# RM-Zhang/SGCDet

Hardware: AMD Instinct MI355X
Metric: scenes/sec (40-view ScanNet volume) at 1/2/4/8 MI355X; mAP@0.25 parity (higher is better)
Workload: dtype f32 (neck/head conv: 3xbf16-split MFMA, fp32 accumulate, ~1e-5 of fp32; wide 3x3x3 stride-1 layers through a Winograd F(2,3) transform along z: <= 2e-5 of the tensor scale per layer against the direct fp32 convolution); 1 GPU; cfg2_scannet: 40 views x 256 ch, images 256x320, FPN maps 64x80/32x40/16x20, D=12, voxels 40x40x16, top-k [800, 6400], neck 3-scale -> ScanNetImVoxelHeadV2; occupancy=predicted, masked_tail=False, input_layout=nchw, scenes_in_flight_per_gpu=4, launch=one hipGraph replay per scene (device-side pair counts, no host read-back)

## Files before the change

sgcdet_amd/csrc/conv3d.hip:

```cpp
#include "conv_common.hpp"
#include "tuning.hpp"

namespace sgc {
int g_conv_products = 3;


__global__ __launch_bounds__(256) void zero_fill_kernel(float4 *__restrict__ p, int64_t n4) {
  for (int64_t i = (int64_t)blockIdx.x * blockDim.x + threadIdx.x; i < n4; i += (int64_t)gridDim.x * blockDim.x)
    p[i] = make_float4(0.f, 0.f, 0.f, 0.f);
}
static int zero_fill(float *y, int64_t n, hipStream_t st) {
  const int64_t n4 = n / 4;
  const int g = (int)((n4 + 255) / 256 < 2048 ? (n4 + 255) / 256 : 2048);
  hipLaunchKernelGGL(zero_fill_kernel, dim3(g > 0 ? g : 1), dim3(256), 0, st, reinterpret_cast<float4 *>(y), n4);
  return check_launch("zero_fill_kernel");
}

static int halo_brick_shape(int gx, int gy, int gz) {
  if (g_tune_halo_brick == 2) return 2;
  if (g_tune_halo_brick == 0 && gz >= 16 && gx % 8 == 0 && gy % 8 == 0 && gz % 4 == 0) return 2;
  if (gz >= 16 && (g_tune_halo_brick == 0 || g_tune_halo_brick == 3)) return 0;
  if (gz >= 8) return 1;
  return 2;
}
// ... 134 lines not shown

static int pick_split_steps(const ConvParams &p, int mb, int nb, int target_blocks, int *steps_per) {
  const int total = (p.transposed ? 1 : p.taps) * (p.Cin / BK);
  *steps_per = total;
  if (p.two_d) return 1;
  if (!p.transposed && p.taps == 1) return 1;
  if (!g_tune_split_free) {
    const int k = pick_splitk(p, mb, nb, target_blocks);
    *steps_per = total / k;
    return k;
  }
  const int64_t tiles = (int64_t)mb * nb * (p.transposed ? 8 : 1);
  int64_t want = target_blocks / (tiles > 0 ? tiles : 1);
  if (want > total / g_tune_split_min_steps) want = total / g_tune_split_min_steps;
  if (want > g_tune_split_max) want = g_tune_split_max;
  if (want <= 1) return 1;
  const int per = (total + (int)want - 1) / (int)want;
  *steps_per = per;
  return (total + per - 1) / per;
}

static int conv_finish(const ConvParams &p, int64_t OV, hipStream_t st) {
  if (p.splitk <= 1) return SGC_OK;
  if (p.Cout % 4) return set_error(SGC_EUNSUP, "conv3d: split-K path needs Cout %% 4 == 0");
  const int64_t total4 = OV * p.Cout / 4;
  const int g = (int)((total4 + 255) / 256 < 4096 ? (total4 + 255) / 256 : 4096);
  hipLaunchKernelGGL(conv_epilogue_kernel, dim3(g), dim3(256), 0, st, p.y, p.scale, p.shift, p.residual, total4,
                     p.Cout / 4, p.relu, (const float *)p.ws, p.splitk, p.act_scale, p.act_c0, p.act_c1);
  return check_launch("conv_epilogue_kernel");
}

static ConvPlan plan_conv(const ConvParams &p, int64_t OV, bool masked) {
  ConvPlan pl = {};
  pl.family = kConvTile; pl.splitk = 1;
  const bool halo = g_tune_conv_halo && !p.transposed && p.ksize == 3 && p.stride == 1 && p.Cout >= g_tune_halo_min_cout;
  const bool narrow_n = g_tune_halo_narrow && p.Cout <= 64;
  const bool narrow_32 = g_tune_halo_narrow >= 1 && g_tune_halo_narrow != 64 && p.Cout <= 32;
  const auto brick = [&pl](ConvFamily f, int bx, int by, int bz, int bn) { pl.family = f; pl.bx = bx; pl.by = by; pl.bz = bz; pl.bn = bn; };
  int small = 0;
  if (!p.transposed && p.ksize == 1 && p.stride == 1 && !p.two_d && rows_gemm_supported(p.Cin, p.Cout, 0, 0, OV, p.Cin)) {
    pl.family = kConvRowsGemm;
    return pl;
  } else if (halo && !p.two_d && p.M >= g_tune_halo_min_m) {
    const int shape = halo_brick_shape(p.gx, p.gy, p.gz), bn = narrow_32 ? 32 : narrow_n ? 64 : 128;
    if (shape == 0) brick(kConvHalo, 4, 4, 16, bn);
    else if (shape == 1) brick(kConvHalo, 4, 8, 8, bn);
    else brick(kConvHalo, 8, 8, 4, bn);
  } else if (halo && !p.two_d && !masked && (small = halo_small_grid(p.gx, p.gy, p.gz, p.Cout)) != 0) {
    if (small == 1) brick(kConvHaloGrid, 10, 10, 4, 64);
    else brick(kConvHaloGrid, 6, 12, 4, 64);
  } else if (halo && g_tune_halo_2d && p.two_d && p.wz_Z > 0 && p.gy >= 8 && p.gz >= 8) {
    const int J = p.wz_Z / 2;
    const bool stack = !narrow_n && p.w_group_images == J && p.gx == 4 * J && p.wz_Z % 4 == 0;
    const bool fit4 = stack && J % 4 == 0 && p.M >= g_tune_halo_min_m, fit2 = stack && (J == 2 || fit4);
    const auto rows = [&p](int bx, int by, int bz) { return (int64_t)ceil_div(p.gx, bx) * ceil_div(p.gy, by) * ceil_div(p.gz, bz) * 256; };
    const bool small = fit2 && (!fit4 || g_tune_wz_brick == 2 || (g_tune_wz_brick == 0 && rows(2, 10, 10) < rows(4, 8, 8)));
    if (small) brick(kConvHaloWZ, 2, 10, 10, 128);
    else if (fit4) brick(kConvHaloWZ, 4, 8, 8, 128);
    if (pl.family == kConvHaloWZ && J % pl.bx != 0) pl.unsupported = "conv: a brick of the virtual Winograd stack must hold images of one position";
    else if (pl.family != kConvHaloWZ) pl.unsupported = "conv: the virtual Winograd stack needs Z / 2 = 2 or a multiple of 4 (and then halo_min_m stack rows) and > 64 output channels";
  } else if (halo && g_tune_halo_2d && p.two_d && p.wz_Z == 0 && p.M >= g_tune_halo_min_m && p.gy >= 8 && p.gz >= 8) {
    if ((g_tune_halo_2d == 2 || p.w_group_images > 0) && !narrow_n && p.gx % 4 == 0 && (p.w_group_images == 0 || p.w_group_images % 4 == 0))
      brick(kConvHalo2D, 4, 8, 8, 128);
    else if (p.w_group_images > 0) pl.unsupported = "conv: grouped 2-D form needs groups of a multiple of 4 images and > 64 output channels";
    else brick(kConvHalo2D, 1, 16, 16, narrow_n ? 64 : 128);
  } else if (p.w_group_images > 0 || p.wz_Z > 0) {
    pl.unsupported = "conv: the grouped 2-D form runs on the halo kernel only (stack too small?)";
  }
  if (pl.unsupported) return pl;
  if (pl.family == kConvTile) {
    pl.bn = p.Cout <= 64 ? 64 : 128;
    pl.splitk = pick_split_steps(p, ceil_div(p.M, BM), ceil_div(p.Cout, pl.bn), g_tune_split_target, &pl.steps_per);
  } else {
    pl.splitk = halo_splitk(ceil_div(p.gx, pl.bx) * ceil_div(p.gy, pl.by) * ceil_div(p.gz, pl.bz), ceil_div(p.Cout, pl.bn), p.Cin / BK);
    if (pl.family == kConvHaloWZ && p.M >= g_tune_halo_min_m) pl.splitk = 1;
  }
  pl.ws_floats = pl.splitk > 1 ? (int64_t)pl.splitk * OV * p.Cout : 0;
  return pl;
}

static int conv_split_begin(ConvParams &p, int64_t OV, hipStream_t st) {
  if (p.splitk <= 1) return SGC_OK;
  if (p.Cout % 4) return set_error(SGC_EUNSUP, "conv3d: split-K path needs Cout %% 4 == 0");
  if (p.ws && p.ws_floats >= (int64_t)p.splitk * OV * p.Cout) {
    p.ws_stride = OV * p.Cout;
    return SGC_OK;
  }
  p.ws = nullptr;
  return zero_fill(p.y, OV * p.Cout, st);
}

// ... 226 lines not shown
```

sgcdet_amd/csrc/conv3d_halo.hpp:

```cpp
#pragma once
#include "conv_common.hpp"
#include "mma.hpp"
#include "diag.hpp"
#include "tuning.hpp"

namespace sgc {

__host__ __device__ constexpr int halo_pitch(int BZ) { return BZ == 8 ? 12 : BZ == 10 ? 13 : BZ + 2; }
__host__ __device__ constexpr size_t halo_tab_offset(int lrows, int mrows = 256, int bnv = 128) {
  const size_t planes = (size_t)(2 * lrows + 2 * 2 * bnv) * LDKH * sizeof(uint16_t);
  const size_t stage = (size_t)mrows * (bnv + 8) * sizeof(float);
  return planes > stage ? planes : stage;
}

template <int BX, int BY, int BZ, int BNV = 128, int NP = 3, bool TD = false, bool STG = true, bool WZ = false>
__global__ __launch_bounds__(512) void conv3d_halo_bf16x3_kernel(const ConvParamsB p) {
  static_assert(!WZ || TD, "the virtual Winograd stack is a 2-D form");
  constexpr int NTAP = TD ? 9 : 27, XO = TD ? 0 : 1;
  constexpr int WNV = BNV >= 64 ? 2 : 1, WMV = 8 / WNV;
  constexpr int NVOX = BX * BY * BZ, MROWS = (NVOX + 32 * WMV - 1) / (32 * WMV) * (32 * WMV);
  constexpr int RT = MROWS / (32 * WMV);
  constexpr unsigned short kPadRow = 0x8000;
  static_assert(MROWS <= 512, "one table entry per thread");
  constexpr int TN = BNV / (32 * WNV), WCOL = BNV / WNV;
  constexpr int HX = BX + 2 * XO, HY = BY + 2, HZ = BZ + 2, HROWS = HX * HY * HZ;
  constexpr int HZP = halo_pitch(BZ), LROWS = HX * HY * HZP;
  constexpr int NT = 512;
  constexpr int NA = (HROWS * 8 + NT - 1) / NT;
  constexpr int A_PLANE = LROWS * LDKH, B_PLANE = BNV * LDKH;
  extern __shared__ __attribute__((aligned(16))) unsigned char smem_h[];
  __bf16 *A_hi = reinterpret_cast<__bf16 *>(smem_h), *A_lo = A_hi + A_PLANE;
  __bf16 *Bbase = A_lo + A_PLANE;
  unsigned short *vox_tab = reinterpret_cast<unsigned short *>(smem_h + halo_tab_offset(LROWS, MROWS, MROWS > 256 ? BNV : 128));

  const int tid = threadIdx.x, lane = tid & 63, wid = tid >> 6;
  const int wm = wid / WNV, wn = wid % WNV;
  const int nby = (p.gy + BY - 1) / BY, nbz = (p.gz + BZ - 1) / BZ;
  int bid = blockIdx.x;
  const int bk = bid % nbz; bid /= nbz;
  const int bj = bid % nby; const int bi = bid / nby;
  const int X0 = bi * BX, Y0 = bj * BY, Z0 = bk * BZ;
  const int n0 = blockIdx.y * BNV;
  const int nchunks = p.Cin / BK;
  const int per = (nchunks + p.splitk - 1) / p.splitk;
  const int c_lo = blockIdx.z * per, c_hi = min(nchunks, c_lo + per);
  if (c_lo >= c_hi) return;

  for (int t = wid; t < MROWS / 32; t += NT / 64) {
    const int j = lane & 31;
    const int r = t * 32 + j, rv = r < NVOX ? r : 0;
    const int x = rv / (BY * BZ), y = (rv / BZ) % BY, z = rv % BZ;
    const int res = (((x + XO) * HY + (y + 1)) * HZP + (z + 1)) & 15;
    unsigned same = 0, mine = 0;
#pragma unroll
    for (int q = 0; q < 16; ++q) {
      const unsigned m = (unsigned)__ballot(res == q);
      if (res == q) same = m;
      if ((j & 15) == q) mine = m;
    }
    const unsigned below = (1u << j) - 1u;
    const int rank = __popc(same & below);
    const bool slot_empty = __popc(mine) < (j >> 4) + 1;
    const unsigned left = (unsigned)__ballot(rank >= 2), empty = (unsigned)__ballot(slot_empty);
    const unsigned short val = r < NVOX ? (unsigned short)r : kPadRow;
    unsigned short *tab = vox_tab + t * 32, *tmp = vox_tab + MROWS + (wid & 7) * 32;
    if (lane < 32) {
      if (rank < 2) tab[rank * 16 + res] = val;
      else tmp[__popc(left & below)] = val;
    }
    asm volatile("s_waitcnt lgkmcnt(0)" ::: "memory");
    if (lane < 32 && slot_empty) tab[j] = tmp[__popc(empty & below)];
  }
  __syncthreads();
  const int fr = lane & 31, fh = lane >> 5;
  int arow[RT];
#pragma unroll
  for (int i = 0; i < RT; ++i) {
    const int r = vox_tab[(wm * RT + i) * 32 + fr] & 0x7fff;
    const int x = r / (BY * BZ), y = (r / BZ) % BY, z = r % BZ;
    arow[i] = ((x + XO) * HY + (y + 1)) * HZP + (z + 1);
  }
  bool wave_live = true;
  if (p.out_mask) {
    bool mine = false;
#pragma unroll
    for (int i = 0; i < RT; ++i) {
      const int r = vox_tab[(wm * RT + i) * 32 + fr];
      const int x = X0 + r / (BY * BZ), y = Y0 + (r / BZ) % BY, z = Z0 + r % BZ;
      if (!(r & kPadRow) && x < p.gx && y < p.gy && z < p.gz) mine |= p.out_mask[((int64_t)x * p.gy + y) * p.gz + z] != 0;
    }
    wave_live = __ballot(mine) != 0ull;
    if (!__syncthreads_or(wave_live ? 1 : 0)) {
      if (p.splitk > 1 && !p.ws) return;
      for (int e = tid; e < NVOX * (BNV / 4); e += NT) {
        const int rl = e / (BNV / 4), c4 = e - rl * (BNV / 4);
        const int col = n0 + c4 * 4;
        if (col >= p.Cout) continue;
        const int x = X0 + rl / (BY * BZ), y = Y0 + (rl / BZ) % BY, z = Z0 + rl % BZ;
        if (x >= p.gx || y >= p.gy || z >= p.gz) continue;
        const int64_t orow = ((int64_t)x * p.gy + y) * p.gz + z;
        for (int q = 0; q < 4 && col + q < p.Cout; ++q) {
          float v = 0.f;
          if (p.splitk > 1) { p.ws[(int64_t)blockIdx.z * p.ws_stride + orow * p.Cout + col + q] = 0.f; continue; }
          v = v * (p.scale ? p.scale[col + q] : 1.f) + (p.shift ? p.shift[col + q] : 0.f);
          if (p.relu == 2) v = relu_nan(v);
          if (p.residual) v += p.residual[orow * p.Cout + col + q];
          if (p.relu == 1) v = relu_nan(v);
          if (p.act_scale) v = act_col(v, col + q, p.act_c0, p.act_c1, *p.act_scale);
          p.y[orow * p.Cout + col + q] = v;
        }
      }
      return;
    }
  }
  const int bc = tid & 3, rs16 = (tid >> 2) & 15;
  const int bn = 16 * wid + (rs16 >> 2) + 4 * (rs16 & 3);
  const bool bn_ok = tid < BNV * 4 && n0 + bn < p.Cout;

  f32x16 acc[RT][TN];
#pragma unroll
  for (int i = 0; i < RT; ++i)
#pragma unroll
    for (int j = 0; j < TN; ++j)
#pragma unroll
      for (int k = 0; k < 16; ++k) acc[i][j][k] = 0.f;
  SGC_HALO_STAMP(0);

  float4 ra[NA], rw[WZ ? NA : 1];
  uint4 rbh, rbl;
  constexpr unsigned OOB = 0xfffffff0u;
  const __amdgpu_buffer_rsrc_t xr = __builtin_amdgcn_make_buffer_rsrc(
      const_cast<float *>(p.x), 0, (int)(unsigned)((int64_t)(WZ ? p.wz_Z : p.ix) * p.iy * p.iz * p.Cin * 4), 0x00020000);
  const int w_bytes = (int)(unsigned)((int64_t)NTAP * p.Cout * p.Cin * 2);
  const int64_t w_set = (TD && p.w_group_images > 0) ? (int64_t)(X0 / p.w_group_images) * NTAP * p.Cout * p.Cin : 0;
  const __amdgpu_buffer_rsrc_t whr = __builtin_amdgcn_make_buffer_rsrc(const_cast<__bf16 *>(p.w_hi + w_set), 0, w_bytes, 0x00020000);
  const __amdgpu_buffer_rsrc_t wlr = __builtin_amdgcn_make_buffer_rsrc(const_cast<__bf16 *>(p.w_lo + w_set), 0, w_bytes, 0x00020000);
  unsigned aoff[NA], aoffb[WZ ? NA : 1];
#pragma unroll
  for (int i = 0; i < NA; ++i) {
    const int idx = i * NT + tid;
    const int row = idx >> 3, c4 = idx & 7;
    const int hz = row % HZ, hy = (row / HZ) % HY, hx = row / (HZ * HY);
    const int gx = X0 + hx - XO, gy = Y0 + hy - 1, gz = Z0 + hz - 1;
    const bool in = row < HROWS && gx >= 0 && gx < p.ix && gy >= 0 && gy < p.iy && gz >= 0 && gz < p.iz;
    if constexpr (WZ) {
      const int J = p.wz_Z >> 1, kpos = X0 / J, j = gx - kpos * J;
      const int za = kpos == 0 ? 2 * j - 1 : kpos == 2 ? 2 * j + 1 : 2 * j;
      const int zb = kpos <= 1 ? 2 * j + 1 : kpos == 2 ? 2 * j : 2 * j + 2;
      const unsigned col = (unsigned)((gy * p.iz + gz) * p.wz_Z);
      aoff[i] = in && za >= 0 ? ((col + (unsigned)za) * (unsigned)p.Cin + c4 * 4) * 4u : OOB;
      aoffb[i] = in && zb < p.wz_Z ? ((col + (unsigned)zb) * (unsigned)p.Cin + c4 * 4) * 4u : OOB;
    } else {
      aoff[i] = in ? ((unsigned)((gx * p.iy + gy) * p.iz + gz) * (unsigned)p.Cin + c4 * 4) * 4u : OOB;
    }
  }
  const float wz_sign = WZ && (X0 / max(p.wz_Z >> 1, 1)) == 1 ? 1.f : -1.f;
  const unsigned boff = bn_ok ? (unsigned)((n0 + bn) * p.Cin + bc * 8) * 2u : OOB;
  auto load_A = [&](int cc) {
// ... 54 lines not shown
    const int dx = TD ? XO : tap / 9, dy = (tap / 3) % 3, dz = tap % 3;
    return ((dx - XO) * HY + (dy - 1)) * HZP + (dz - 1);
  };
  struct Frag { bf16x8 ah[RT], al[RT], bh[TN], bl[TN]; };
  auto read_A = [&](Frag &f, int toff, int kk) {
#pragma unroll
    for (int i = 0; i < RT; ++i) {
      const int o = (arow[i] + toff) * LDKH + fh * 8 + kk * 16;
      f.ah[i] = *reinterpret_cast<const bf16x8 *>(A_hi + o);
      if constexpr (NP == 3) f.al[i] = *reinterpret_cast<const bf16x8 *>(A_lo + o);
    }
  };
  auto read_B = [&](Frag &f, int buf, int kk) {
    const __bf16 *b = Bbase + buf * 2 * B_PLANE + (wn * WCOL + fr) * LDKH + fh * 8 + kk * 16;
#pragma unroll
    for (int j = 0; j < TN; ++j) {
      f.bh[j] = *reinterpret_cast<const bf16x8 *>(b + j * 32 * LDKH);
      if constexpr (NP == 3) f.bl[j] = *reinterpret_cast<const bf16x8 *>(b + B_PLANE + j * 32 * LDKH);
    }
  };
  auto mfma_half = [&](const Frag &f) {
    if constexpr ((SGC_HALO_SKIP & 32) != 0) {
#pragma unroll
      for (int i = 0; i < RT; ++i) asm volatile("" ::"v"(f.ah[i]), "v"(f.al[i]));
#pragma unroll
      for (int j = 0; j < TN; ++j) asm volatile("" ::"v"(f.bh[j]), "v"(f.bl[j]));
      return;
    }
#pragma unroll
    for (int i = 0; i < RT; ++i)
#pragma unroll
      for (int j = 0; j < TN; ++j) acc[i][j] = mma_split<NP>(f.ah[i], f.al[i], f.bh[j], f.bl[j], acc[i][j]);
  };
  const int steps_total = (c_hi - c_lo) * NTAP;
  auto step_tap = [&](int st) { return st % NTAP; };
  auto step_cc = [&](int st) { return c_lo + st / NTAP; };

  if constexpr (STG) {
    load_A(c_lo);
    load_B(0, c_lo);
    split_A();
    store_A();
    store_B(0);
    if (steps_total > 1) load_B(step_tap(1), step_cc(1));
    __syncthreads();
    Frag P = {}, Q = {};
    constexpr int SKIP = SGC_HALO_SKIP;
    if (wave_live) { read_A(P, tap_off(0), 0); read_B(P, 0, 0); }
    int g = 0;
    for (int cc = c_lo; cc < c_hi; ++cc) {
#pragma unroll
      for (int tap = 0; tap < NTAP; ++tap, ++g) {
        const bool last_tap = tap == NTAP - 1;
        const bool more = g + 1 < steps_total;
        if (wave_live) {
          if (!(SKIP & 16) || g == 0) read_A(Q, tap_off(tap), 1);
          if (!(SKIP & 8) || g == 0) read_B(Q, g & 1, 1);
        }
        if (!(SKIP & 2) && more) store_B((g + 1) & 1);
        if (!(SKIP & 4) && g + 2 < steps_total) load_B(step_tap(g + 2), step_cc(g + 2));
        if (!(SKIP & 64) && tap == NTAP - 3 && cc + 1 < c_hi) load_A(cc + 1);
        if (wave_live) mfma_half(P);
        if (!(SKIP & 64) && last_tap && cc + 1 < c_hi) split_A();
        if (!(SKIP & 1)) __syncthreads();
        __builtin_amdgcn_sched_barrier(0);
        if (wave_live && !last_tap) {
          if (!(SKIP & 16)) read_A(P, tap_off(tap + 1), 0);
          if (!(SKIP & 8)) read_B(P, (g + 1) & 1, 0);
        }
        if (!(SKIP & 64) && last_tap && cc + 1 < c_hi) store_A();
        if (wave_live) mfma_half(Q);
// ... 14 lines not shown
    store_B(0);
    __syncthreads();
    Frag P = {}, Q = {};
    read_A(P, tap_off(0), 0);
    for (int cc = c_lo; cc < c_hi; ++cc) {
      for (int tap = 0; tap < NTAP; ++tap, ++g) {
        const bool last_tap = tap == NTAP - 1;
        if (!(SKIP & 4) && g + 1 < steps_total) load_B(step_tap(g + 1), step_cc(g + 1));
        if (tap == NTAP - 3 && cc + 1 < c_hi) load_A(cc + 1);
        const int toff = tap_off(tap);
        if (wave_live) {
          if (!(SKIP & 8) || g == 0) read_B(P, g & 1, 0);
          if (!(SKIP & 16) || g == 0) read_A(Q, toff, 1);
          if (!(SKIP & 8) || g == 0) read_B(Q, g & 1, 1);
          mfma_half(P);
          mfma_half(Q);
          if (!last_tap && (!(SKIP & 16) || g == 0)) read_A(P, tap_off(tap + 1), 0);
        }
        if (!(SKIP & 2) && g + 1 < steps_total) store_B((g + 1) & 1);
        if (last_tap && cc + 1 < c_hi) split_A();
        if (!(SKIP & 1)) __syncthreads();
      }
      if (cc + 1 < c_hi) {
        store_A();
        __syncthreads();
        if (wave_live && (!(SKIP & 16))) read_A(P, tap_off(0), 0);
      }
    }
  }
  SGC_HALO_STAMP(2);
  if constexpr ((SGC_HALO_SKIP & 128) != 0) { if (p.relu != 77) return; }

  if ((p.Cout & 3) == 0 && (p.splitk == 1 || p.ws)) {
    constexpr int LDC = BNV + 8;
    float *cs = reinterpret_cast<float *>(smem_h);
    if constexpr (STG) __syncthreads();
#pragma unroll
    for (int i = 0; i < RT; ++i)
#pragma unroll
      for (int j = 0; j < TN; ++j)
#pragma unroll
        for (int k = 0; k < 16; ++k)
          cs[(wm * (RT * 32) + i * 32 + (k & 3) + 8 * (k >> 2) + 4 * (lane >> 5)) * LDC + wn * WCOL + j * 32 + (lane & 31)] = acc[i][j][k];
    __syncthreads();
    constexpr int C4 = BNV / 4;
    for (int e = tid; e < MROWS * C4; e += NT) {
      const int rl = e / C4, c4 = e - rl * C4;
      const int col = n0 + c4 * 4;
      if (col >= p.Cout) continue;
      const int r = vox_tab[rl];
      if (r & kPadRow) continue;
      const int x = X0 + r / (BY * BZ), y = Y0 + (r / BZ) % BY, z = Z0 + r % BZ;
      if (x >= p.gx || y >= p.gy || z >= p.gz) continue;
      const int64_t orow = ((int64_t)x * p.gy + y) * p.gz + z;
      float4 v = *reinterpret_cast<const float4 *>(cs + rl * LDC + c4 * 4);
      if (p.splitk > 1) {
        *reinterpret_cast<float4 *>(p.ws + (int64_t)blockIdx.z * p.ws_stride + orow * p.Cout + col) = v;
        continue;
      }
      if (p.scale) {
        const float4 sc4 = *reinterpret_cast<const float4 *>(p.scale + col);
        v.x *= sc4.x; v.y *= sc4.y; v.z *= sc4.z; v.w *= sc4.w;
      }
      if (p.shift) {
        const float4 sh4 = *reinterpret_cast<const float4 *>(p.shift + col);
        v.x += sh4.x; v.y += sh4.y; v.z += sh4.z; v.w += sh4.w;
      }
      if (p.relu == 2) v = relu_nan(v);
      if (p.residual) {
        const float4 r4 = *reinterpret_cast<const float4 *>(p.residual + orow * p.Cout + col);
        v.x += r4.x; v.y += r4.y; v.z += r4.z; v.w += r4.w;
      }
      if (p.relu == 1) v = relu_nan(v);
      if (p.act_scale) v = act_col4(v, col, p.act_c0, p.act_c1, *p.act_scale);
      *reinterpret_cast<float4 *>(p.y + orow * p.Cout + col) = v;
    }
    return;
  }

#pragma unroll
  for (int i = 0; i < RT; ++i)
#pragma unroll
    for (int j = 0; j < TN; ++j) {
      const int col = n0 + wn * WCOL + j * 32 + (lane & 31);
      if (col >= p.Cout) continue;
      const float sc = p.scale ? p.scale[col] : 1.f, sh = p.shift ? p.shift[col] : 0.f;
#pragma unroll
      for (int k = 0; k < 16; ++k) {
        const int r = vox_tab[(wm * RT + i) * 32 + (k & 3) + 8 * (k >> 2) + 4 * (lane >> 5)];
        const int x = X0 + r / (BY * BZ), y = Y0 + (r / BZ) % BY, z = Z0 + r % BZ;
        if ((r & kPadRow) || x >= p.gx || y >= p.gy || z >= p.gz) continue;
        const int64_t orow = ((int64_t)x * p.gy + y) * p.gz + z;
        float *dst = p.y + orow * p.Cout + col;
        if (p.splitk > 1) {
          if (p.ws) p.ws[(int64_t)blockIdx.z * p.ws_stride + orow * p.Cout + col] = acc[i][j][k];
          else atomicAdd(dst, acc[i][j][k]);
        } else {
          float v = acc[i][j][k] * sc + sh;
          if (p.relu == 2) v = relu_nan(v);
          if (p.residual) v += p.residual[orow * p.Cout + col];
          if (p.relu == 1) v = relu_nan(v);
          if (p.act_scale) v = act_col(v, col, p.act_c0, p.act_c1, *p.act_scale);
          *dst = v;
        }
      }
    }
}


template <int BX, int BY, int BZ, int BNV, int NP, bool TD, bool STG, bool WZ = false>
static int launch_halo_k(ConvParamsB &p, hipStream_t st) {
#if defined(SGC_HALO_STAMPS)
  p.stamps = g_halo_stamp_buf;
#endif
  constexpr int LROWS = (TD ? BX : BX + 2) * (BY + 2) * halo_pitch(BZ);
  constexpr int RGRAN = BNV >= 64 ? 128 : 256;
  constexpr int MROWS = (BX * BY * BZ + RGRAN - 1) / RGRAN * RGRAN;
  const size_t smem = halo_tab_offset(LROWS, MROWS, MROWS > 256 ? BNV : 128) + (MROWS + 256) * sizeof(uint16_t);
  static_assert(halo_tab_offset(LROWS, MROWS, MROWS > 256 ? BNV : 128) + (MROWS + 256) * sizeof(uint16_t) <= 160 * 1024, "brick does not fit the LDS");
  static std::atomic<uint64_t> attr_done{0};
  ensure_dynamic_lds((const void *)conv3d_halo_bf16x3_kernel<BX, BY, BZ, BNV, NP, TD, STG, WZ>, (int)smem, attr_done);
  const int bricks = ceil_div(p.gx, BX) * ceil_div(p.gy, BY) * ceil_div(p.gz, BZ);
  const int nb = ceil_div(p.Cout, BNV);
  hipLaunchKernelGGL((conv3d_halo_bf16x3_kernel<BX, BY, BZ, BNV, NP, TD, STG, WZ>), dim3(bricks, nb, p.splitk), dim3(512), smem, st, p);
  return check_launch("conv3d_halo_bf16x3_kernel");
}

template <int BX, int BY, int BZ, int BNV = 128, bool TD = false, bool WZ = false>
static int launch_halo(ConvParamsB &p, hipStream_t st) {
  if constexpr (!WZ) {
    if (g_conv_products == 3) {
      if (!g_tune_halo_stagger || BX * BY * BZ > 256) return launch_halo_k<BX, BY, BZ, BNV, 3, TD, false>(p, st);
      return launch_halo_k<BX, BY, BZ, BNV, 3, TD, true>(p, st);
    }
  }
  return with_products(g_conv_products, [&](auto np) { return launch_halo_k<BX, BY, BZ, BNV, np(), TD, true, WZ>(p, st); });
}

int launch_halo_z4(ConvParamsB &p, const ConvPlan &pl, hipStream_t st);
int launch_halo_2d(ConvParamsB &p, const ConvPlan &pl, hipStream_t st);
}
```

sgcdet_amd/csrc/conv3d_halo_2d.hip:

```cpp
#include "conv3d_halo.hpp"

namespace sgc {
int launch_halo_2d(ConvParamsB &p, const ConvPlan &pl, hipStream_t st) {
  if (pl.family == kConvHaloWZ)
    return pl.bx == 2 ? launch_halo<2, 10, 10, 128, true, true>(p, st) : launch_halo<4, 8, 8, 128, true, true>(p, st);
  if (pl.bx == 4) return launch_halo<4, 8, 8, 128, true>(p, st);
  return pl.bn == 64 ? launch_halo<1, 16, 16, 64, true>(p, st) : launch_halo<1, 16, 16, 128, true>(p, st);
}
}
```

sgcdet_amd/csrc/conv_common.hpp:

```cpp
#pragma once
#include "common.hpp"

namespace sgc {
extern int g_conv_products;

bool rows_gemm_supported(int K, int N, int hm_cm, int hm_S, int64_t rows, int64_t ldx);
int device_cus();
int rows_gemm_launch(const float *x, int64_t ldx, const uint16_t *w_hi, const uint16_t *w_lo, const float *scale,
                     const float *shift, const float *residual, void *y, const int32_t *m_dev, int M, int K, int N, int relu,
                     int hm_S, int hm_cm, int hm_bf16, hipStream_t st, float *zero_row = nullptr);
bool rows_gemm_gather_supported(int K, int N, int64_t x_rows, int64_t rows);
int rows_gemm_gather_launch(const float *x, int64_t x_rows, const float *gw, const int32_t *go, const uint16_t *w_hi, const uint16_t *w_lo,
                            const float *shift, float *y, const int32_t *m_dev, int M, int K, int N, hipStream_t st);

struct ConvParams {
  const float *x;
  const float *w;
  const float *scale;
  const float *shift;
  const float *residual;
  float *y;
  int Cin, Cout;
  int ix, iy, iz;
  int gx, gy, gz;
// ... 12 lines not shown
  int two_d;
  unsigned long long *stamps;
  int xcd_deal;
  int wz_Z;
  int w_group_images;
  float *zero_row;
  const float *act_scale;
  int act_c0, act_c1;
  int hm_bf16;
  int hm_S, hm_cm;
};

__device__ __forceinline__ float act_col(float v, int col, int c0, int c1, float s) { return (col >= c0 && col < c1) ? expf(v * s) : v; }
__device__ __forceinline__ float4 act_col4(float4 v, int col, int c0, int c1, float s) {
  if (c1 <= c0) return v;
  return make_float4(act_col(v.x, col, c0, c1, s), act_col(v.y, col + 1, c0, c1, s), act_col(v.z, col + 2, c0, c1, s), act_col(v.w, col + 3, c0, c1, s));
}

constexpr int BM = 128, BK = 32, LDK = BK + 4;

typedef unsigned int u32x4 __attribute__((ext_vector_type(4)));
constexpr int LDKH = BK + 8;
constexpr int igemm_tile_lds_bytes(int bn) { return 2 * (2 * BM + 2 * bn) * LDKH * 2; }

struct ConvParamsB : ConvParams {
  const __bf16 *w_hi, *w_lo;
};

enum ConvFamily { kConvRowsGemm, kConvHalo, kConvHaloGrid, kConvHalo2D, kConvHaloWZ, kConvTile };
struct ConvPlan {
  ConvFamily family;
  int bx, by, bz;
  int bn;
  int splitk, steps_per;
  int64_t ws_floats;
  const char *unsupported;
};

int launch_igemm_f32(const ConvParams &p, bool narrow, dim3 grid, hipStream_t st);
void launch_igemm(const ConvParamsB &p, bool narrow, dim3 grid, size_t smem, hipStream_t st);
int launch_halo(ConvParamsB &p, const ConvPlan &pl, hipStream_t st);
}
```

sgcdet_amd/csrc/mma.hpp:

```cpp
#pragma once
#include <hip/hip_runtime.h>
#include <type_traits>

namespace sgc {

typedef float f32x16 __attribute__((ext_vector_type(16)));
typedef __bf16 bf16x8 __attribute__((ext_vector_type(8)));
typedef __bf16 bf16x4 __attribute__((ext_vector_type(4)));
typedef _Float16 f16x8 __attribute__((ext_vector_type(8)));

template <int NP>
__device__ __forceinline__ __bf16 op_hi(float v) {
  if constexpr (NP == 2) {
    const float c = v != v ? v : fminf(fmaxf(v, -65504.f), 65504.f);
    return __builtin_bit_cast(__bf16, (_Float16)c);
  } else {
    return (__bf16)v;
  }
}
template <int NP>
__device__ __forceinline__ __bf16 op_lo(float v, __bf16 hi) {
  if constexpr (NP == 3) return (__bf16)(v - (float)hi);
  else return __builtin_bit_cast(__bf16, (unsigned short)0);
}
template <int NP>
__device__ __forceinline__ void split4(const float (&v)[4], bf16x4 &h, bf16x4 &l) {
  bf16x4 h4, l4;
#pragma unroll
  for (int e = 0; e < 4; ++e) {
    const __bf16 hb = op_hi<NP>(v[e]);
    h4[e] = hb;
    l4[e] = op_lo<NP>(v[e], hb);
  }
  h = h4;
  l = l4;
}
__host__ __device__ constexpr int acc_row(int k) { return (k & 3) + 8 * (k >> 2); }
template <int NP>
__device__ __forceinline__ f32x16 mma_hh(bf16x8 a, bf16x8 b, f32x16 c) {
  if constexpr (NP == 2)
    return __builtin_amdgcn_mfma_f32_32x32x16_f16(__builtin_bit_cast(f16x8, a), __builtin_bit_cast(f16x8, b), c, 0, 0, 0);
  else
    return __builtin_amdgcn_mfma_f32_32x32x16_bf16(a, b, c, 0, 0, 0);
}
template <int NP>
__device__ __forceinline__ f32x16 mma_split(const bf16x8 &ah, const bf16x8 &al, const bf16x8 &bh, const bf16x8 &bl, f32x16 c) {
  if constexpr (NP == 3) {
    c = __builtin_amdgcn_mfma_f32_32x32x16_bf16(al, bh, c, 0, 0, 0);
    c = __builtin_amdgcn_mfma_f32_32x32x16_bf16(ah, bl, c, 0, 0, 0);
  }
  return mma_hh<NP>(ah, bh, c);
}

template <class F>
inline auto with_products(int products, F &&f) {
  if (products == 1) return f(std::integral_constant<int, 1>{});
  if (products == 2) return f(std::integral_constant<int, 2>{});
  return f(std::integral_constant<int, 3>{});
}

}
```

sgcdet_amd/csrc/tuning.hpp:

```cpp
#pragma once

#define SGC_TUNING_KNOBS(X)                                                                                                   \
                                                              \
  X("fwd_variant", g_tune_fwd_variant, 1, "0: block-barrier kernel, 1: wave-private kernel (when the shape allows)")         \
  X("fwd_spl", g_tune_fwd_spl, 1, "samples per lane in phase 1 of the wave kernel (1, 2, 4)")                                \
  X("tile_nw", g_tune_tile_nw, 0, "waves per workgroup (8 or 16); 0: by LDS footprint")                                      \
  X("tile_depth_lds", g_tune_tile_depth_lds, -1, ">= 0 overrides the caller's depth_in_lds")                                 \
  X("tile_diag", g_tune_tile_diag, 0, "timing experiments only (1 no compute, 2 no fill); inert without SGC_DIAG=1")         \
  X("tile_nbuf", g_tune_tile_nbuf, 0, "value-window buffers (2 needs heads per workgroup > 1); 0: one")                      \
  X("tile_xcd", g_tune_tile_xcd, -1, "1: camera n on XCD n % 8, 0: head h on XCD h, -1: 1 at Cm = 32, 0 at Cm = 16")          \
  X("tile_hg", g_tune_tile_hg, 0, "heads per workgroup; 0: one")                                                             \
  X("tile_ds", g_tune_tile_ds, 1, "1: one window test for value and depth where the windows coincide")                       \
  X("bwd_tile_diag", g_tune_bwd_tile_diag, 0, "timing experiments only; inert without SGC_DIAG=1")                           \
                                           \
  X("compact2", g_tune_compact2, 1, "1: two-launch segment form of sgc_compact_pairs, 0: the five kernels")                  \
  X("view_depth", g_tune_pq_depth, 4, "pair rows in flight per lane in view_attend / view_mean (1 | 2 | 4 | 8)")             \
  X("view_group", g_tune_view_group, 1, "0: the per-camera loops in view_mean / view_attend")                                \
  X("topk_multi_min", g_tune_topk_multi_min, 32769, "fewest candidates for the many-workgroup top-k")                        \
                                                                                               \
  X("rows_gemm", g_tune_rows_gemm, 1, "0: every row GEMM on the tile implicit-GEMM kernel")                                  \
  X("rows_diag", g_tune_rows_diag, 0, "timing experiments only (bit 0 no stores, 1 no loads, 2 no MFMA); needs SGC_DIAG=1")  \
  X("rows_cu_pct", g_tune_rows_cu_pct, 100, "persistent row GEMM: share of the CUs it occupies")                             \
  X("rows_depth", g_tune_rows_depth, 1, "8-wave form: 2 = two tiles in flight ahead, anything else = one")                   \
                                                                \
  X("conv_halo", g_tune_conv_halo, 1, "3x3x3 stride-1 layers: 0 tile kernel, 1 halo-resident kernel")                        \
  X("halo_min_cout", g_tune_halo_min_cout, 16, "fewest output channels for the halo kernel")                                 \
  X("halo_min_m", g_tune_halo_min_m, 2048, "fewest output voxels for the halo kernel")                                       \
  X("halo_brick", g_tune_halo_brick, 0, "0: brick by grid, 1: prefer 4x8x8, 2: force 8x8x4, 3: 4x4x16 at depth >= 16")       \
  X("halo_small", g_tune_halo_small, 1, "1: whole-grid bricks for the 10x10x4 / 12x12x4 grids at Cout >= 512")               \
  X("halo_narrow", g_tune_halo_narrow, 1, "1: 64- and 32-column tiles for few output channels, 64: never below 64, 0: 128")  \
  X("halo_2d", g_tune_halo_2d, 1, "3x3 layers over an image stack: 1 bricks of 16 x 16 pixels, 2 of 4 images x 8 x 8, 0 tile kernel") \
  X("wz_brick", g_tune_wz_brick, 0, "Winograd-z stack: 0 the brick with fewer matrix rows, 1: 4 images x 8 x 8, 2: 2 images x 10 x 10 (where each fits)") \
  X("halo_split_target", g_tune_halo_split_target, 192, "halo kernel: channel slices are split until a launch has this many workgroups") \
  X("halo_wave_fix", g_tune_halo_wave_fix, 1, "one more split on a small CU overflow: 1 latency geometry only, 2 always")    \
  X("split_target", g_tune_split_target, 512, "tile kernel: the reduction is split until a launch has this many workgroups") \
  X("split_free", g_tune_split_free, 1, "tile kernel: 1 splits of whole K steps, 0 of whole tap groups")                     \
  X("split_min_steps", g_tune_split_min_steps, 8, "tile kernel: fewest K steps of a split (>= 1)")                           \
  X("split_max", g_tune_split_max, 32, "tile kernel: most splits (>= 1)")                                                    \
                                            \
  X("conv_waves", g_tune_conv_waves, 8, "tile kernel: 4 or 8 waves per 128 x 128 tile")                                      \
  X("igemm_xcd", g_tune_igemm_xcd, 0, "tile kernel: XCD deal of the split / transposed layers (ConvParams.xcd_deal)")        \
  X("halo_stagger", g_tune_halo_stagger, 1, "halo kernel: 1 barrier at mid-tap (software-pipelined), 0 lockstep")            \
  X("wgrad_waves", g_tune_wgrad_waves, 8, "weight-gradient tile kernel: 4 or 8 waves")                                       \
  X("wgrad_halo", g_tune_wgrad_halo, 1, "3x3x3 stride-1 weight gradient: 1 double-buffered halo form, 2 single, 0 tile kernel")

namespace sgc {
#define SGC_KNOB_DECLARE(key, var, def, doc) extern int var;
SGC_TUNING_KNOBS(SGC_KNOB_DECLARE)
#undef SGC_KNOB_DECLARE
}
```

Baseline: 542.4 scenes/sec.

## Run Winograd-z halo bricks on 16x16x32 MFMA with reworked LDS layout

Adds a 16x16x32 bf16 MFMA variant of the pipelined halo conv kernel for the Winograd-z stacked bricks and makes it the default through a new wz_mfma knob. It changes the voxel-to-row seating table for 8 residues, the LDS pitch and K stride to avoid bank conflicts, the fragment loads, the per-product MFMA interleave with B prefetch, and the accumulator store paths. The smaller MFMA tile is meant to cut instruction latency and register pressure and to improve LDS access patterns on these bricks. In exchange it issues more MFMA instructions per tile and reorders the accumulation, which gives last-bit differences in the results.

```diff
diff --git a/sgcdet_amd/csrc/conv3d.hip b/sgcdet_amd/csrc/conv3d.hip
--- a/sgcdet_amd/csrc/conv3d.hip
+++ b/sgcdet_amd/csrc/conv3d.hip
@@ -190,7 +190,7 @@
 
 static ConvPlan plan_conv(const ConvParams &p, int64_t OV, bool masked) {
   ConvPlan pl = {};
-  pl.family = kConvTile; pl.splitk = 1;
+  pl.family = kConvTile; pl.splitk = 1; pl.mfma = 32;
   const bool halo = g_tune_conv_halo && !p.transposed && p.ksize == 3 && p.stride == 1 && p.Cout >= g_tune_halo_min_cout;
   const bool narrow_n = g_tune_halo_narrow && p.Cout <= 64;
   const bool narrow_32 = g_tune_halo_narrow >= 1 && g_tune_halo_narrow != 64 && p.Cout <= 32;
@@ -215,6 +215,7 @@
     const bool small = fit2 && (!fit4 || g_tune_wz_brick == 2 || (g_tune_wz_brick == 0 && rows(2, 10, 10) < rows(4, 8, 8)));
     if (small) brick(kConvHaloWZ, 2, 10, 10, 128);
     else if (fit4) brick(kConvHaloWZ, 4, 8, 8, 128);
+    pl.mfma = g_tune_wz_mfma == 32 ? 32 : 16;
     if (pl.family == kConvHaloWZ && J % pl.bx != 0) pl.unsupported = "conv: a brick of the virtual Winograd stack must hold images of one position";
     else if (pl.family != kConvHaloWZ) pl.unsupported = "conv: the virtual Winograd stack needs Z / 2 = 2 or a multiple of 4 (and then halo_min_m stack rows) and > 64 output channels";
   } else if (halo && g_tune_halo_2d && p.two_d && p.wz_Z == 0 && p.M >= g_tune_halo_min_m && p.gy >= 8 && p.gz >= 8) {
diff --git a/sgcdet_amd/csrc/conv3d_halo.hpp b/sgcdet_amd/csrc/conv3d_halo.hpp
--- a/sgcdet_amd/csrc/conv3d_halo.hpp
+++ b/sgcdet_amd/csrc/conv3d_halo.hpp
@@ -6,16 +6,19 @@
 
 namespace sgc {
 
-__host__ __device__ constexpr int halo_pitch(int BZ) { return BZ == 8 ? 12 : BZ == 10 ? 13 : BZ + 2; }
-__host__ __device__ constexpr size_t halo_tab_offset(int lrows, int mrows = 256, int bnv = 128) {
-  const size_t planes = (size_t)(2 * lrows + 2 * 2 * bnv) * LDKH * sizeof(uint16_t);
+__host__ __device__ constexpr int halo_pitch(int BZ, int MF = 32) { return BZ == 8 ? 12 : BZ == 10 ? (MF == 16 ? 14 : 13) : BZ + 2; }
+__host__ __device__ constexpr int halo_ldk(int MF) { return MF == 16 ? BK + 16 : LDKH; }
+__host__ __device__ constexpr size_t halo_tab_offset(int lrows, int mrows = 256, int bnv = 128, int ldk = LDKH) {
+  const size_t planes = (size_t)(2 * lrows + 2 * 2 * bnv) * ldk * sizeof(uint16_t);
   const size_t stage = (size_t)mrows * (bnv + 8) * sizeof(float);
   return planes > stage ? planes : stage;
 }
 
-template <int BX, int BY, int BZ, int BNV = 128, int NP = 3, bool TD = false, bool STG = true, bool WZ = false>
+template <int BX, int BY, int BZ, int BNV = 128, int NP = 3, bool TD = false, bool STG = true, bool WZ = false, int MF = 32>
 __global__ __launch_bounds__(512) void conv3d_halo_bf16x3_kernel(const ConvParamsB p) {
   static_assert(!WZ || TD, "the virtual Winograd stack is a 2-D form");
+  static_assert(MF == 32 || (MF == 16 && WZ && STG && BNV == 128 && BX * BY * BZ <= 256), "the 16x16x32 form: pipelined Winograd bricks only");
+  constexpr int LDKH = halo_ldk(MF);
   constexpr int NTAP = TD ? 9 : 27, XO = TD ? 0 : 1;
   constexpr int WNV = BNV >= 64 ? 2 : 1, WMV = 8 / WNV;
   constexpr int NVOX = BX * BY * BZ, MROWS = (NVOX + 32 * WMV - 1) / (32 * WMV) * (32 * WMV);
@@ -24,14 +27,14 @@
   static_assert(MROWS <= 512, "one table entry per thread");
   constexpr int TN = BNV / (32 * WNV), WCOL = BNV / WNV;
   constexpr int HX = BX + 2 * XO, HY = BY + 2, HZ = BZ + 2, HROWS = HX * HY * HZ;
-  constexpr int HZP = halo_pitch(BZ), LROWS = HX * HY * HZP;
+  constexpr int HZP = halo_pitch(BZ, MF), LROWS = HX * HY * HZP;
   constexpr int NT = 512;
   constexpr int NA = (HROWS * 8 + NT - 1) / NT;
   constexpr int A_PLANE = LROWS * LDKH, B_PLANE = BNV * LDKH;
   extern __shared__ __attribute__((aligned(16))) unsigned char smem_h[];
   __bf16 *A_hi = reinterpret_cast<__bf16 *>(smem_h), *A_lo = A_hi + A_PLANE;
   __bf16 *Bbase = A_lo + A_PLANE;
-  unsigned short *vox_tab = reinterpret_cast<unsigned short *>(smem_h + halo_tab_offset(LROWS, MROWS, MROWS > 256 ? BNV : 128));
+  unsigned short *vox_tab = reinterpret_cast<unsigned short *>(smem_h + halo_tab_offset(LROWS, MROWS, MROWS > 256 ? BNV : 128, LDKH));
 
   const int tid = threadIdx.x, lane = tid & 63, wid = tid >> 6;
   const int wm = wid / WNV, wn = wid % WNV;
@@ -46,26 +49,33 @@
   const int c_lo = blockIdx.z * per, c_hi = min(nchunks, c_lo + per);
   if (c_lo >= c_hi) return;
 
+  constexpr int RES = MF == 16 ? 8 : 16, RANKS = 32 / RES;
+  const auto seat = [](int k, int q) {
+    if constexpr (MF == 16) return (k >> 1) * 16 + ((k & 1) ? 4 + q : q < 4 ? q : q + 8);
+    else return k * 16 + q;
+  };
   for (int t = wid; t < MROWS / 32; t += NT / 64) {
     const int j = lane & 31;
     const int r = t * 32 + j, rv = r < NVOX ? r : 0;
     const int x = rv / (BY * BZ), y = (rv / BZ) % BY, z = rv % BZ;
-    const int res = (((x + XO) * HY + (y + 1)) * HZP + (z + 1)) & 15;
+    const int res = (((x + XO) * HY + (y + 1)) * HZP + (z + 1)) & (RES - 1);
+    const int ji = j & 15, jb = MF == 16 && ji >= 4 && ji < 12;
+    const int sq = MF == 16 ? (jb ? ji - 4 : ji < 4 ? ji : ji - 8) : ji, sk = MF == 16 ? 2 * (j >> 4) + jb : j >> 4;
     unsigned same = 0, mine = 0;
 #pragma unroll
-    for (int q = 0; q < 16; ++q) {
+    for (int q = 0; q < RES; ++q) {
       const unsigned m = (unsigned)__ballot(res == q);
       if (res == q) same = m;
-      if ((j & 15) == q) mine = m;
+      if (sq == q) mine = m;
     }
     const unsigned below = (1u << j) - 1u;
     const int rank = __popc(same & below);
-    const bool slot_empty = __popc(mine) < (j >> 4) + 1;
-    const unsigned left = (unsigned)__ballot(rank >= 2), empty = (unsigned)__ballot(slot_empty);
+    const bool slot_empty = __popc(mine) < sk + 1;
+    const unsigned left = (unsigned)__ballot(rank >= RANKS), empty = (unsigned)__ballot(slot_empty);
     const unsigned short val = r < NVOX ? (unsigned short)r : kPadRow;
     unsigned short *tab = vox_tab + t * 32, *tmp = vox_tab + MROWS + (wid & 7) * 32;
     if (lane < 32) {
-      if (rank < 2) tab[rank * 16 + res] = val;
+      if (rank < RANKS) tab[seat(rank, res)] = val;
       else tmp[__popc(left & below)] = val;
     }
     asm volatile("s_waitcnt lgkmcnt(0)" ::: "memory");
@@ -73,10 +83,12 @@
   }
   __syncthreads();
   const int fr = lane & 31, fh = lane >> 5;
-  int arow[RT];
-#pragma unroll
-  for (int i = 0; i < RT; ++i) {
-    const int r = vox_tab[(wm * RT + i) * 32 + fr] & 0x7fff;
+  constexpr int RT16 = 2 * RT, TN16 = BNV / (16 * WNV);
+  const int fr16 = lane & 15, fq = lane >> 4;
+  int arow[MF == 16 ? RT16 : RT];
+#pragma unroll
+  for (int i = 0; i < (MF == 16 ? RT16 : RT); ++i) {
+    const int r = (MF == 16 ? vox_tab[wm * RT * 32 + i * 16 + fr16] : vox_tab[(wm * RT + i) * 32 + fr]) & 0x7fff;
     const int x = r / (BY * BZ), y = (r / BZ) % BY, z = r % BZ;
     arow[i] = ((x + XO) * HY + (y + 1)) * HZP + (z + 1);
   }
@@ -114,16 +126,23 @@
     }
   }
   const int bc = tid & 3, rs16 = (tid >> 2) & 15;
-  const int bn = 16 * wid + (rs16 >> 2) + 4 * (rs16 & 3);
+  const int bn = MF == 16 ? 16 * wid + 2 * (rs16 & 3) + ((rs16 >> 2) & 1) + 8 * (rs16 >> 3) : 16 * wid + (rs16 >> 2) + 4 * (rs16 & 3);
   const bool bn_ok = tid < BNV * 4 && n0 + bn < p.Cout;
 
-  f32x16 acc[RT][TN];
-#pragma unroll
-  for (int i = 0; i < RT; ++i)
-#pragma unroll
-    for (int j = 0; j < TN; ++j)
+  f32x16 acc[MF == 16 ? 1 : RT][MF == 16 ? 1 : TN];
+  f32x4 acc16[MF == 16 ? RT16 : 1][MF == 16 ? TN16 : 1];
+#pragma unroll
+  for (int i = 0; i < (MF == 16 ? 1 : RT); ++i)
+#pragma unroll
+    for (int j = 0; j < (MF == 16 ? 1 : TN); ++j)
 #pragma unroll
       for (int k = 0; k < 16; ++k) acc[i][j][k] = 0.f;
+#pragma unroll
+  for (int i = 0; i < (MF == 16 ? RT16 : 1); ++i)
+#pragma unroll
+    for (int j = 0; j < (MF == 16 ? TN16 : 1); ++j)
+#pragma unroll
+      for (int k = 0; k < 4; ++k) acc16[i][j][k] = 0.f;
   SGC_HALO_STAMP(0);
 
   float4 ra[NA], rw[WZ ? NA : 1];
@@ -244,11 +263,81 @@
 #pragma unroll
       for (int j = 0; j < TN; ++j) acc[i][j] = mma_split<NP>(f.ah[i], f.al[i], f.bh[j], f.bl[j], acc[i][j]);
   };
+  struct FragA16 { bf16x8 h[2], l[2]; };
+  struct FragB16 { bf16x8 h[TN16], l[TN16]; };
+  auto read_A16 = [&](FragA16 &f, int toff, int half) {
+#pragma unroll
+    for (int i = 0; i < 2; ++i) {
+      const int o = (arow[MF == 16 ? 2 * half + i : 0] + toff) * LDKH + fq * 8;
+      f.h[i] = *reinterpret_cast<const bf16x8 *>(A_hi + o);
+      if constexpr (NP == 3) f.l[i] = *reinterpret_cast<const bf16x8 *>(A_lo + o);
+    }
+  };
+  auto read_B16 = [&](FragB16 &f, int buf, int j) {
+    const __bf16 *b = Bbase + buf * 2 * B_PLANE + (wn * WCOL + j * 16 + fr16) * LDKH + fq * 8;
+    f.h[j] = *reinterpret_cast<const bf16x8 *>(b);
+    if constexpr (NP == 3) f.l[j] = *reinterpret_cast<const bf16x8 *>(b + B_PLANE);
+  };
+  auto mfma16_half = [&](const FragA16 &a, int half, FragB16 &b, int next_buf) {
+#pragma unroll
+    for (int j = 0; j < TN16; ++j) {
+      f32x4 &c0 = acc16[MF == 16 ? 2 * half : 0][MF == 16 ? j : 0], &c1 = acc16[MF == 16 ? 2 * half + 1 : 0][MF == 16 ? j : 0];
+      c0 = mma_split_one<NP, 0>(a.h[0], a.l[0], b.h[j], b.l[j], c0);
+      c1 = mma_split_one<NP, 0>(a.h[1], a.l[1], b.h[j], b.l[j], c1);
+      c0 = mma_split_one<NP, 1>(a.h[0], a.l[0], b.h[j], b.l[j], c0);
+      c1 = mma_split_one<NP, 1>(a.h[1], a.l[1], b.h[j], b.l[j], c1);
+      c0 = mma_split_one<NP, 2>(a.h[0], a.l[0], b.h[j], b.l[j], c0);
+      c1 = mma_split_one<NP, 2>(a.h[1], a.l[1], b.h[j], b.l[j], c1);
+      if (next_buf >= 0) read_B16(b, next_buf, j);
+    }
+  };
   const int steps_total = (c_hi - c_lo) * NTAP;
   auto step_tap = [&](int st) { return st % NTAP; };
   auto step_cc = [&](int st) { return c_lo + st / NTAP; };
 
-  if constexpr (STG) {
+  if constexpr (MF == 16) {
+    load_A(c_lo);
+    load_B(0, c_lo);
+    split_A();
+    store_A();
+    store_B(0);
+    if (steps_total > 1) load_B(step_tap(1), step_cc(1));
+    __syncthreads();
+    FragA16 P = {}, Q = {};
+    FragB16 B = {};
+    if (wave_live) {
+      read_A16(P, tap_off(0), 0);
+#pragma unroll
+      for (int j = 0; j < TN16; ++j) read_B16(B, 0, j);
+    }
+    int g = 0;
+    for (int cc = c_lo; cc < c_hi; ++cc) {
+#pragma unroll
+      for (int tap = 0; tap < NTAP; ++tap, ++g) {
+        const bool last_tap = tap == NTAP - 1;
+        if (wave_live) read_A16(Q, tap_off(tap), 1);
+        if (g + 1 < steps_total) store_B((g + 1) & 1);
+        if (g + 2 < steps_total) load_B(step_tap(g + 2), step_cc(g + 2));
+        if (tap == NTAP - 3 && cc + 1 < c_hi) load_A(cc + 1);
+        if (wave_live) mfma16_half(P, 0, B, -1);
+        if (last_tap && cc + 1 < c_hi) split_A();
+        __syncthreads();
+        __builtin_amdgcn_sched_barrier(0);
+        if (wave_live && !last_tap) read_A16(P, tap_off(tap + 1), 0);
+        if (last_tap && cc + 1 < c_hi) store_A();
+        if (wave_live) mfma16_half(Q, 1, B, last_tap ? -1 : (g + 1) & 1);
+        __builtin_amdgcn_sched_barrier(0);
+      }
+      if (cc + 1 < c_hi) {
+        __syncthreads();
+        if (wave_live) {
+          read_A16(P, tap_off(0), 0);
+#pragma unroll
+          for (int j = 0; j < TN16; ++j) read_B16(B, g & 1, j);
+        }
+      }
+    }
+  } else if constexpr (STG) {
     load_A(c_lo);
     load_B(0, c_lo);
     split_A();
@@ -329,9 +418,18 @@
   if constexpr ((SGC_HALO_SKIP & 128) != 0) { if (p.relu != 77) return; }
 
   if ((p.Cout & 3) == 0 && (p.splitk == 1 || p.ws)) {
-    constexpr int LDC = BNV + 8;
+    constexpr int LDC = MF == 16 ? BNV + 4 : BNV + 8;
     float *cs = reinterpret_cast<float *>(smem_h);
     if constexpr (STG) __syncthreads();
+    if constexpr (MF == 16) {
+#pragma unroll
+      for (int i = 0; i < RT16; ++i)
+#pragma unroll
+        for (int j = 0; j < TN16; ++j)
+#pragma unroll
+          for (int k = 0; k < 4; ++k)
+            cs[(wm * (RT * 32) + i * 16 + acc16_row(lane) + k) * LDC + wn * WCOL + j * 16 + fr16] = acc16[i][j][k];
+    } else {
 #pragma unroll
     for (int i = 0; i < RT; ++i)
 #pragma unroll
@@ -339,6 +437,7 @@
 #pragma unroll
         for (int k = 0; k < 16; ++k)
           cs[(wm * (RT * 32) + i * 32 + (k & 3) + 8 * (k >> 2) + 4 * (lane >> 5)) * LDC + wn * WCOL + j * 32 + (lane & 31)] = acc[i][j][k];
+    }
     __syncthreads();
     constexpr int C4 = BNV / 4;
     for (int e = tid; e < MROWS * C4; e += NT) {
@@ -375,6 +474,36 @@
     return;
   }
 
+  const auto store_one = [&](int tab_row, int col, float sc, float sh, float a) {
+    const int r = vox_tab[tab_row];
+    const int x = X0 + r / (BY * BZ), y = Y0 + (r / BZ) % BY, z = Z0 + r % BZ;
+    if ((r & kPadRow) || x >= p.gx || y >= p.gy || z >= p.gz) return;
+    const int64_t orow = ((int64_t)x * p.gy + y) * p.gz + z;
+    float *dst = p.y + orow * p.Cout + col;
+    if (p.splitk > 1) {
+      if (p.ws) p.ws[(int64_t)blockIdx.z * p.ws_stride + orow * p.Cout + col] = a;
+      else atomicAdd(dst, a);
+    } else {
+      float v = a * sc + sh;
+      if (p.relu == 2) v = relu_nan(v);
+      if (p.residual) v += p.residual[orow * p.Cout + col];
+      if (p.relu == 1) v = relu_nan(v);
+      if (p.act_scale) v = act_col(v, col, p.act_c0, p.act_c1, *p.act_scale);
+      *dst = v;
+    }
+  };
+  if constexpr (MF == 16) {
+#pragma unroll
+    for (int i = 0; i < RT16; ++i)
+#pragma unroll
+      for (int j = 0; j < TN16; ++j) {
+        const int col = n0 + wn * WCOL + j * 16 + fr16;
+        if (col >= p.Cout) continue;
+        const float sc = p.scale ? p.scale[col] : 1.f, sh = p.shift ? p.shift[col] : 0.f;
+#pragma unroll
+        for (int k = 0; k < 4; ++k) store_one(wm * RT * 32 + i * 16 + acc16_row(lane) + k, col, sc, sh, acc16[i][j][k]);
+      }
+  } else {
 #pragma unroll
   for (int i = 0; i < RT; ++i)
 #pragma unroll
@@ -402,28 +531,29 @@
         }
       }
     }
+  }
 }
 
 
-template <int BX, int BY, int BZ, int BNV, int NP, bool TD, bool STG, bool WZ = false>
+template <int BX, int BY, int BZ, int BNV, int NP, bool TD, bool STG, bool WZ = false, int MF = 32>
 static int launch_halo_k(ConvParamsB &p, hipStream_t st) {
 #if defined(SGC_HALO_STAMPS)
   p.stamps = g_halo_stamp_buf;
 #endif
-  constexpr int LROWS = (TD ? BX : BX + 2) * (BY + 2) * halo_pitch(BZ);
+  constexpr int LROWS = (TD ? BX : BX + 2) * (BY + 2) * halo_pitch(BZ, MF);
   constexpr int RGRAN = BNV >= 64 ? 128 : 256;
   constexpr int MROWS = (BX * BY * BZ + RGRAN - 1) / RGRAN * RGRAN;
-  const size_t smem = halo_tab_offset(LROWS, MROWS, MROWS > 256 ? BNV : 128) + (MROWS + 256) * sizeof(uint16_t);
-  static_assert(halo_tab_offset(LROWS, MROWS, MROWS > 256 ? BNV : 128) + (MROWS + 256) * sizeof(uint16_t) <= 160 * 1024, "brick does not fit the LDS");
+  const size_t smem = halo_tab_offset(LROWS, MROWS, MROWS > 256 ? BNV : 128, halo_ldk(MF)) + (MROWS + 256) * sizeof(uint16_t);
+  static_assert(halo_tab_offset(LROWS, MROWS, MROWS > 256 ? BNV : 128, halo_ldk(MF)) + (MROWS + 256) * sizeof(uint16_t) <= 160 * 1024, "brick does not fit the LDS");
   static std::atomic<uint64_t> attr_done{0};
-  ensure_dynamic_lds((const void *)conv3d_halo_bf16x3_kernel<BX, BY, BZ, BNV, NP, TD, STG, WZ>, (int)smem, attr_done);
+  ensure_dynamic_lds((const void *)conv3d_halo_bf16x3_kernel<BX, BY, BZ, BNV, NP, TD, STG, WZ, MF>, (int)smem, attr_done);
   const int bricks = ceil_div(p.gx, BX) * ceil_div(p.gy, BY) * ceil_div(p.gz, BZ);
   const int nb = ceil_div(p.Cout, BNV);
-  hipLaunchKernelGGL((conv3d_halo_bf16x3_kernel<BX, BY, BZ, BNV, NP, TD, STG, WZ>), dim3(bricks, nb, p.splitk), dim3(512), smem, st, p);
+  hipLaunchKernelGGL((conv3d_halo_bf16x3_kernel<BX, BY, BZ, BNV, NP, TD, STG, WZ, MF>), dim3(bricks, nb, p.splitk), dim3(512), smem, st, p);
   return check_launch("conv3d_halo_bf16x3_kernel");
 }
 
-template <int BX, int BY, int BZ, int BNV = 128, bool TD = false, bool WZ = false>
+template <int BX, int BY, int BZ, int BNV = 128, bool TD = false, bool WZ = false, int MF = 32>
 static int launch_halo(ConvParamsB &p, hipStream_t st) {
   if constexpr (!WZ) {
     if (g_conv_products == 3) {
@@ -431,7 +561,7 @@
       return launch_halo_k<BX, BY, BZ, BNV, 3, TD, true>(p, st);
     }
   }
-  return with_products(g_conv_products, [&](auto np) { return launch_halo_k<BX, BY, BZ, BNV, np(), TD, true, WZ>(p, st); });
+  return with_products(g_conv_products, [&](auto np) { return launch_halo_k<BX, BY, BZ, BNV, np(), TD, true, WZ, MF>(p, st); });
 }
 
 int launch_halo_z4(ConvParamsB &p, const ConvPlan &pl, hipStream_t st);
diff --git a/sgcdet_amd/csrc/conv3d_halo_2d.hip b/sgcdet_amd/csrc/conv3d_halo_2d.hip
--- a/sgcdet_amd/csrc/conv3d_halo_2d.hip
+++ b/sgcdet_amd/csrc/conv3d_halo_2d.hip
@@ -2,6 +2,8 @@
 
 namespace sgc {
 int launch_halo_2d(ConvParamsB &p, const ConvPlan &pl, hipStream_t st) {
+  if (pl.family == kConvHaloWZ && pl.mfma == 16)
+    return pl.bx == 2 ? launch_halo<2, 10, 10, 128, true, true, 16>(p, st) : launch_halo<4, 8, 8, 128, true, true, 16>(p, st);
   if (pl.family == kConvHaloWZ)
     return pl.bx == 2 ? launch_halo<2, 10, 10, 128, true, true>(p, st) : launch_halo<4, 8, 8, 128, true, true>(p, st);
   if (pl.bx == 4) return launch_halo<4, 8, 8, 128, true>(p, st);
diff --git a/sgcdet_amd/csrc/conv_common.hpp b/sgcdet_amd/csrc/conv_common.hpp
--- a/sgcdet_amd/csrc/conv_common.hpp
+++ b/sgcdet_amd/csrc/conv_common.hpp
@@ -68,6 +68,7 @@
   ConvFamily family;
   int bx, by, bz;
   int bn;
+  int mfma;
   int splitk, steps_per;
   int64_t ws_floats;
   const char *unsupported;
diff --git a/sgcdet_amd/csrc/mma.hpp b/sgcdet_amd/csrc/mma.hpp
--- a/sgcdet_amd/csrc/mma.hpp
+++ b/sgcdet_amd/csrc/mma.hpp
@@ -52,6 +52,29 @@
   return mma_hh<NP>(ah, bh, c);
 }
 
+typedef float f32x4 __attribute__((ext_vector_type(4)));
+__host__ __device__ constexpr int acc16_row(int lane) { return 4 * (lane >> 4); }
+template <int NP>
+__device__ __forceinline__ f32x4 mma_hh(bf16x8 a, bf16x8 b, f32x4 c) {
+  if constexpr (NP == 2)
+    return __builtin_amdgcn_mfma_f32_16x16x32_f16(__builtin_bit_cast(f16x8, a), __builtin_bit_cast(f16x8, b), c, 0, 0, 0);
+  else
+    return __builtin_amdgcn_mfma_f32_16x16x32_bf16(a, b, c, 0, 0, 0);
+}
+template <int NP, int PROD>
+__device__ __forceinline__ f32x4 mma_split_one(const bf16x8 &ah, const bf16x8 &al, const bf16x8 &bh, const bf16x8 &bl, f32x4 c) {
+  if constexpr (PROD == 2) return mma_hh<NP>(ah, bh, c);
+  else if constexpr (NP != 3) return c;
+  else if constexpr (PROD == 0) return __builtin_amdgcn_mfma_f32_16x16x32_bf16(al, bh, c, 0, 0, 0);
+  else return __builtin_amdgcn_mfma_f32_16x16x32_bf16(ah, bl, c, 0, 0, 0);
+}
+template <int NP>
+__device__ __forceinline__ f32x4 mma_split(const bf16x8 &ah, const bf16x8 &al, const bf16x8 &bh, const bf16x8 &bl, f32x4 c) {
+  c = mma_split_one<NP, 0>(ah, al, bh, bl, c);
+  c = mma_split_one<NP, 1>(ah, al, bh, bl, c);
+  return mma_split_one<NP, 2>(ah, al, bh, bl, c);
+}
+
 template <class F>
 inline auto with_products(int products, F &&f) {
   if (products == 1) return f(std::integral_constant<int, 1>{});
diff --git a/sgcdet_amd/csrc/tuning.hpp b/sgcdet_amd/csrc/tuning.hpp
--- a/sgcdet_amd/csrc/tuning.hpp
+++ b/sgcdet_amd/csrc/tuning.hpp
@@ -31,6 +31,7 @@
   X("halo_narrow", g_tune_halo_narrow, 1, "1: 64- and 32-column tiles for few output channels, 64: never below 64, 0: 128")  \
   X("halo_2d", g_tune_halo_2d, 1, "3x3 layers over an image stack: 1 bricks of 16 x 16 pixels, 2 of 4 images x 8 x 8, 0 tile kernel") \
   X("wz_brick", g_tune_wz_brick, 0, "Winograd-z stack: 0 the brick with fewer matrix rows, 1: 4 images x 8 x 8, 2: 2 images x 10 x 10 (where each fits)") \
+  X("wz_mfma", g_tune_wz_mfma, 16, "Winograd-z bricks: MFMA shape, 16 = 16x16x32, 32 = 32x32x16 (last-bit differences; each value deterministic)") \
   X("halo_split_target", g_tune_halo_split_target, 192, "halo kernel: channel slices are split until a launch has this many workgroups") \
   X("halo_wave_fix", g_tune_halo_wave_fix, 1, "one more split on a small CU overflow: 1 latency geometry only, 2 always")    \
   X("split_target", g_tune_split_target, 512, "tile kernel: the reduction is split until a launch has this many workgroups") \
```

Result: faster. 557.2 scenes/sec, median of 6 (+2.7%).
